# hanmekim/SceneLib2

Measured on AMD Instinct MI355X. Metric: batched MonoSLAM frames/sec (320x240, 100 feat), higher is better.
Workload: dtype f64

## Files before the change

scenelib2_amd/csrc/sl2_common.hpp:

```cpp
#pragma once
#include <hip/hip_runtime.h>

#include <cstdio>
#include <cstring>
#include <string>
#include <vector>

#include "../../include/scenelib2_amd.h"
#include "sl2_math.hpp"
#include "sl2_seq_arrays.hpp"
#include "sl2_step_plan.hpp"

namespace sl2 {

void set_error(const std::string& s);
const char* hip_err_text(hipError_t e);

#define SL2_HIP(call)                                                                          \
  do {                                                                                         \
    hipError_t _e = (call);                                                                    \
    if (_e != hipSuccess) {                                                                    \
      char _buf[512];                                                                          \
      snprintf(_buf, sizeof(_buf), "%s:%d: %s -> %s", __FILE__, __LINE__, #call, hipGetErrorString(_e)); \
      sl2::set_error(_buf);                                                                    \
      return SL2_ERR_HIP;                                                                      \
    }                                                                                          \
  } while (0)

inline int round_up(int v, int a) { return (v + a - 1) / a * a; }

enum : int {
  FF_ACTIVE = 1,
  FF_SCHEDULED = 2,
  FF_SELECTED = 4,
  FF_SUCCESS = 8,
  FF_VISIBLE = 16,
  FF_USED = 32,
  FF_PARTIAL = 64,
};

constexpr int kMaxParticles = 1024;
constexpr int kSrchSplitDefault = 8;
__host__ __device__ inline int srch_split_default(int width, int height) {
  const int frame_bands = ((width + 31) / 32) * ((height + 15) / 16);
  const int t = frame_bands * kSrchSplitDefault / 150;
  return t > kSrchSplitDefault ? t : kSrchSplitDefault;
}
constexpr int kSrchBigUnits = 16384;
constexpr int kSrchBigSlots = 64;
constexpr int kSrchBigMinBands = 4;
constexpr int kSrchSharedNu = -(1 << 30);
constexpr int kSrchBigEntries = 4;
constexpr int kSrchBigDone = kSrchBigEntries + 4 * kSrchBigUnits;
constexpr int kSrchBigParts = kSrchBigDone + kSrchBigUnits;
constexpr int kSrchBigInts = kSrchBigParts + 8 * kSrchBigUnits;
constexpr int kSeqTimeNominal = 0, kSeqTimeOwed = 1, kSeqTimeUsed = 2, kSeqTimeCatchUp = 3;
constexpr int kSeqCamFku = 0, kSeqCamFkv = 1, kSeqCamU0 = 2, kSeqCamV0 = 3, kSeqCamKd1 = 4, kSeqCamSd = 5;
static_assert(kSeqCamDoubles * sizeof(double) == 64, "one cache line per sequence");
__host__ __device__ inline int srch_unit_bands(int bands) { const int g = (bands + kSrchBigSlots - 1) / kSrchBigSlots; return g > kSrchBigMinBands ? g : kSrchBigMinBands; }
constexpr int kMaxPartial = 4;
enum : int { kPartCount = 0, kPartOrder , kPartUU = 5, kPartVV, kPartRegionValid,
             kPartRegion , kPartInitialised = 12, kPartConverted, kPartDeleted, kPartCreated };
enum : int { kPsActive = 0, kPsLabel , kPsAttempts, kPsNp, kPsMaking };
constexpr int kCholBlock = 32;
constexpr int kPatchPackedOffset = 128;

constexpr int kXcds = 8;
inline int xcd_grid(int tiles, int B) { return tiles * round_up(B, kXcds); }
#if defined(__HIPCC__)
__device__ __forceinline__ bool xcd_map(int tiles, int B, int* seq, int* tile) {
  const int L = blockIdx.x;
  const int xcd = L % kXcds, slot = L / kXcds;
  *seq = (slot / tiles) * kXcds + xcd;
  *tile = slot % tiles;
  return *seq < B;
}
#endif

#if defined(__HIPCC__)
__device__ __forceinline__ CameraParams load_cam(const double* __restrict__ seq_cam, int b, int width, int height) {
  const double* rec = seq_cam + (size_t)b * kSeqCamDoubles;
  CameraParams cam;
  cam.width = width; cam.height = height;
  cam.fku = rec[kSeqCamFku]; cam.fkv = rec[kSeqCamFkv]; cam.u0 = rec[kSeqCamU0]; cam.v0 = rec[kSeqCamV0];
  cam.kd1 = rec[kSeqCamKd1]; cam.sd = (int)rec[kSeqCamSd];
  return cam;
}
#endif

struct KernelTimer {
  std::string name;
  double total_ms = 0.0;
  int64_t launches = 0;
};
struct PendingEvent {
  int timer;
  hipEvent_t start, stop;
};

}

struct sl2_engine : sl2::SeqArrays {
  int device = 0;
  hipStream_t stream = nullptr;
  bool own_stream = false;
  sl2::CameraParams cam;
  sl2_params prm;
  int B = 0;
  int N = 0;
  int ld = 0;
  int nsel_max = 0;
  int mld = 0;
  int nblk_max = 0;
  long long steps_done = 0;
  int chol_variant = 1;
  void* chol_trace = nullptr;
  int build_variant = 1;
  int fwd_variant = 1;
  int ppos = 0;
  int kpart = 1;
  int pcap = 128;
  double* score_map = nullptr;
  int* me_big_list = nullptr;
  int* me_big_count = nullptr;
  bool mapping_used = false;
  int* init_uv = nullptr;
  struct StepGraph { const void* frames; size_t stride; sl2::StepPlan plan; hipGraphExec_t exec; };
  bool graph_mode = false;
  std::vector<StepGraph> step_graphs;
  long long graph_captures = 0;
  int build_split = 0;
  int score_threads = 0;
  int no_ksplit = 0;
  int panel_from = 16;
  int group_from = 13;
  int fwd_group = 8;
  int chol_panel = 8;
  int build_lds_min = 0;
  int search_lds_pad = 0;
  int search_chunk = 0;
  int search_variant = 1;
  int* slots_max_dev = nullptr;
  unsigned long long* slots_mail = nullptr;
  unsigned long long* slots_mail_dev = nullptr;
  unsigned long long* parts_mail = nullptr;
  unsigned long long* parts_mail_dev = nullptr;
  int place_candidates = 0;
  float place_syrk_ms[2] = {0, 0};
  float place_kept_ms[4] = {0, 0, 0, 0};
  float place_worst_ms[3] = {0, 0, 0};
  long long parts_block_step = -1;
  int slots_exact = 0;
  long long slots_exact_step = 0;
  int step_fusion = 1;
  int search_split = sl2::kSrchSplitDefault;
  int* srch_big = nullptr;
  std::vector<sl2_camera> cams_host;
  void* stats_host = nullptr;
  void* stats_host_dev = nullptr;

  void* snap_stage = nullptr;
  void* snap_host = nullptr;
  void* snap_host_dev = nullptr;
  size_t snap_cap = 0;
  unsigned long long snap_ticket = 0;
  void* snapb_stage = nullptr;
  size_t snapb_stage_bytes = 0;
  void* snapb_aux = nullptr;
  void* snapb_aux_host = nullptr;
  void* ovl_lists = nullptr;
  size_t ovl_lists_bytes = 0;
  void* ovl_images = nullptr;
  size_t ovl_images_bytes = 0;
  void* acc_dev = nullptr;
  size_t acc_dev_bytes = 0;
  void* acc_host = nullptr;
  size_t acc_host_bytes = 0;
  void* ckpt_stage = nullptr;
  size_t ckpt_stage_bytes = 0;
  hipEvent_t ckpt_event = nullptr;

  uint8_t* frames_buf = nullptr;
  const uint8_t* cur_frames = nullptr;
  size_t cur_stride = 0;

  bool profiling = false;
  int profile_level = 2;
  std::string profile_focus;
  std::vector<sl2::KernelTimer> timers;
  std::vector<sl2::PendingEvent> pending;
  std::vector<hipEvent_t> event_pool;

  sl2_engine* root = nullptr;
  std::vector<sl2_engine*> groups;
  int group_first = 0;
  hipEvent_t fork_event = nullptr;

  int timer_id(const char* name);
  void prof_begin(int id, hipStream_t st);
  void prof_end(hipStream_t st);
  int fold_events();
  int sync_all();
};

namespace sl2 {

inline const SeqArrays& seq_arrays(const sl2_engine* e) { return *e; }

struct LaunchScope {
  sl2_engine* e;
  bool on;
  size_t slot = 0;
  static bool wanted(const sl2_engine* r, const char* name, bool major) {
    if (!r->profiling) return false;
    if (r->profile_level >= 2) return true;
    if (!major) return false;
    if (r->profile_focus.empty()) return true;
    return r->profile_focus.find(std::string(",") + name + ",") != std::string::npos;
  }
  LaunchScope(sl2_engine* eng, const char* name, bool major = false) : e(eng), on(wanted(eng->root, name, major)) {
    if (on) { e->root->prof_begin(e->root->timer_id(name), e->stream); slot = e->root->pending.size() - 1; }
  }
  ~LaunchScope() {
    if (on) hipEventRecord(e->root->pending[slot].stop, e->stream);
  }
};

int launch_predict(sl2_engine* e);
int launch_feature_prediction(sl2_engine* e);
int launch_select(sl2_engine* e, int n);
int launch_search(sl2_engine* e);
int launch_search_kernel(sl2_engine* e);
int launch_search_score(sl2_engine* e);
int launch_small_front(sl2_engine* e, int n);
int launch_small_back(sl2_engine* e, int save_trajectory, int panel_w);
int launch_update(sl2_engine* e);
int launch_syrk_on(sl2_engine* e, const double* Vt, double* P);
int launch_finalize(sl2_engine* e, int save_trajectory);
int launch_mapping(sl2_engine* e, const TailPlan& tp);
int launch_manual_init(sl2_engine* e, const int* d_uv);
int launch_auto_init(sl2_engine* e);
int launch_compact_slots(sl2_engine* e, int need, bool honour_mask = false);
int checkpoint_refresh_slots(sl2_engine* e);
int checkpoint_drop_graphs(sl2_engine* e);
int checkpoint_enable_mapping(sl2_engine* e);
void release_checkpoint_staging(sl2_engine* e);
int write_grey_image(const char* path, const uint8_t* px, int w, int h);

}
```

scenelib2_amd/csrc/sl2_ekf_update.hip:

```cpp
#include "sl2_common.hpp"
#include "sl2_chol_diag.hpp"

namespace sl2 {

typedef double v4d __attribute__((ext_vector_type(4)));

__device__ __forceinline__ v4d mfma_f64(double a, double b, v4d c) {
  return __builtin_amdgcn_mfma_f64_16x16x4f64(a, b, c, 0, 0, 0);
}

#ifdef SL2_TESTING
#define SL2_EKF_TEST_SECTION 1
#include "sl2_ekf_update_testing.inc"
#undef SL2_EKF_TEST_SECTION
#endif

constexpr int kASBatch = 4;

template <int NQ, int BATCH>
__global__ void __launch_bounds__(1024) k_build_AS(const double* __restrict__ P, const double* __restrict__ f_Hx,
                                                  const double* __restrict__ f_Hy, const double* __restrict__ f_nu,
                                                  const double* __restrict__ f_R, const int* __restrict__ succ_idx,
                                                  const int* __restrict__ m_count, double* __restrict__ At,
                                                  double* __restrict__ St, const int* __restrict__ f_hcol,
                                                  const int* __restrict__ pos_err_any, int N, int ld, int mld) {
  extern __shared__ double sAt[];
  const int b = blockIdx.x;
  const int cnt = m_count[b];
  if (cnt == 0) return;
  const int m = 2 * cnt, mp = (m + 31) / 32 * 32;
  const int t = threadIdx.x;
  double* Ab = At + (size_t)b * mld * ld;
  double* Sb = St + (size_t)b * mld * mld;
  const double* Pb = P + (size_t)b * ld * ld;
  const int* sidx = succ_idx + (size_t)b * N;
  const int* hcol = (pos_err_any[b] != 0) ? f_hcol + (size_t)b * N : nullptr;
  double pc[NQ][7];
#pragma unroll
  for (int q = 0; q < NQ; ++q) {
    const int i = t + q * (int)blockDim.x;
#pragma unroll
    for (int c = 0; c < 7; ++c) pc[q][c] = (i >= ld) ? 0.0 : ((i < 13) ? Pb[(size_t)i * ld + c] : Pb[(size_t)c * ld + i]);
  }
  double hx[7], hy[3], Rn = 0.0;
  int posa = 0;
  if (t < m) {
    const int fa = sidx[t >> 1];
    const size_t fia = (size_t)b * N + fa;
    posa = hcol ? hcol[fa] : 13 + 3 * fa;
#pragma unroll
    for (int c = 0; c < 7; ++c) hx[c] = (hcol && (unsigned)(c - posa) < 3u) ? 0.0 : f_Hx[fia * 14 + (t & 1) * 7 + c];
#pragma unroll
    for (int c = 0; c < 3; ++c) hy[c] = f_Hy[fia * 6 + (t & 1) * 3 + c];
    Rn = f_R[fia];
  }
  const int nbatch = (cnt + BATCH - 1) / BATCH, per = (nbatch + (int)gridDim.y - 1) / (int)gridDim.y;
  const int jbeg = (int)blockIdx.y * per * BATCH;
  const int jend = (jbeg + per * BATCH < cnt) ? jbeg + per * BATCH : cnt;
  for (int j0 = jbeg; j0 < jend; j0 += BATCH) {
    const int nb = (jend - j0 < BATCH) ? jend - j0 : BATCH;
#pragma unroll
    for (int jj = 0; jj < BATCH; ++jj) {
      if (jj < nb) {
        const int f = sidx[j0 + jj];
        const size_t fi = (size_t)b * N + f;
        const int pos = hcol ? hcol[f] : 13 + 3 * f;
#pragma unroll
        for (int q = 0; q < NQ; ++q) {
          const int i = t + q * (int)blockDim.x;
          if (i < ld) {
            double py[3];
#pragma unroll
            for (int c = 0; c < 3; ++c)
              py[c] = Pb[(size_t)(pos + c) * ld + i];
#pragma unroll
            for (int r = 0; r < 2; ++r) {
              double acc = 0.0;
#pragma unroll
              for (int c = 0; c < 7; ++c) acc += pc[q][c] * ((hcol && (unsigned)(c - pos) < 3u) ? 0.0 : f_Hx[fi * 14 + r * 7 + c]);
#pragma unroll
              for (int c = 0; c < 3; ++c) acc += py[c] * f_Hy[fi * 6 + r * 3 + c];
              if (i == ld - 1) acc = f_nu[fi * 2 + r];
              Ab[(size_t)(2 * (j0 + jj) + r) * ld + i] = acc;
              sAt[(2 * jj + r) * ld + i] = acc;
            }
          }
        }
      }
    }
    __syncthreads();
    if (t < mp) {
#pragma unroll
      for (int kk = 0; kk < 2 * BATCH; ++kk) {
        const int k = 2 * j0 + kk;
        if (kk < 2 * nb && (t | 31) >= k) {
          double v = 0.0;
          if (t < m) {
            const double* arow = sAt + kk * ld;
            double acc = 0.0;
#pragma unroll
            for (int c = 0; c < 7; ++c) acc += hx[c] * arow[c];
#pragma unroll
            for (int c = 0; c < 3; ++c) acc += hy[c] * arow[posa + c];
            if (t == k) acc += Rn;
            v = acc;
          }
          Sb[(size_t)k * mld + t] = v;
        }
      }
    }
    __syncthreads();
  }
  if (blockIdx.y != 0) return;
  for (int k = m; k < mp; ++k) {
#pragma unroll
    for (int q = 0; q < NQ; ++q) {
      const int i = t + q * (int)blockDim.x;
      if (i < ld) Ab[(size_t)k * ld + i] = 0.0;
    }
    if (t < mp && (t | 31) >= k) Sb[(size_t)k * mld + t] = (t == k) ? 1.0 : 0.0;
  }
}


#ifdef SL2_TESTING
#define SL2_EKF_TEST_SECTION 3
#include "sl2_ekf_update_testing.inc"
#undef SL2_EKF_TEST_SECTION
#endif


__device__ __forceinline__ double fast_rcp(double p) {
  double r = __builtin_amdgcn_rcp(p);
  r = __builtin_fma(__builtin_fma(-p, r, 1.0), r, r);
  r = __builtin_fma(__builtin_fma(-p, r, 1.0), r, r);
  return r;
}
__device__ __forceinline__ double fast_rsqrt(double p) {
  double y = __builtin_amdgcn_rsq(p);
  y = y * __builtin_fma(-0.5 * p * y, y, 1.5);
  y = y * __builtin_fma(-0.5 * p * y, y, 1.5);
  return y;
}


#ifdef SL2_TESTING
#define SL2_EKF_TEST_SECTION 4
#include "sl2_ekf_update_testing.inc"
#undef SL2_EKF_TEST_SECTION
#endif

#ifdef SL2_TESTING
#define SL2_EKF_TEST_SECTION 5
#include "sl2_ekf_update_testing.inc"
#undef SL2_EKF_TEST_SECTION
#endif

#ifdef SL2_TESTING
#define SL2_EKF_TEST_SECTION 6
#include "sl2_ekf_update_testing.inc"
#undef SL2_EKF_TEST_SECTION
#endif


struct Tile32 {
  v4d f[2][2];
};

__device__ __forceinline__ Tile32 tile_load(const double* __restrict__ Sb, int mld, int k0, int i0, int lo, int hi) {
  Tile32 t;
#pragma unroll
  for (int kt = 0; kt < 2; ++kt)
#pragma unroll
    for (int it = 0; it < 2; ++it)
#pragma unroll
      for (int r = 0; r < 4; ++r) t.f[kt][it][r] = Sb[(size_t)(k0 + 16 * kt + hi + 4 * r) * mld + i0 + 16 * it + lo];
  return t;
}
__device__ __forceinline__ void tile_store(double* __restrict__ Sb, int mld, int k0, int i0, int lo, int hi, const Tile32& t) {
#pragma unroll
  for (int kt = 0; kt < 2; ++kt)
#pragma unroll
    for (int it = 0; it < 2; ++it)
#pragma unroll
      for (int r = 0; r < 4; ++r) Sb[(size_t)(k0 + 16 * kt + hi + 4 * r) * mld + i0 + 16 * it + lo] = t.f[kt][it][r];
}
constexpr int kTileAll = 15, kTileRowsLo = 5, kTileDiag = 11, kTileDiagLo = 1;
__device__ __forceinline__ Tile32 tile_panel(const double* sLinv, const double* __restrict__ Sb, int mld, int o, int i0, int lo,
                                             int hi, int need) {
  double b0[8], b1[8];
#pragma unroll
  for (int s8 = 0; s8 < 8; ++s8) {
    b0[s8] = Sb[(size_t)(o + 4 * s8 + hi) * mld + i0 + lo];
    b1[s8] = (need & 10) ? Sb[(size_t)(o + 4 * s8 + hi) * mld + i0 + 16 + lo] : 0.0;
  }
  Tile32 t;
#pragma unroll
  for (int kt = 0; kt < 2; ++kt)
#pragma unroll
    for (int it = 0; it < 2; ++it) t.f[kt][it] = (v4d){0, 0, 0, 0};
#pragma unroll
  for (int s8 = 0; s8 < 8; ++s8) {
    const int p = 4 * s8 + hi;
    const double a0 = sLinv[p * kLinvPitch + lo], a1 = sLinv[p * kLinvPitch + 16 + lo];
    t.f[0][0] = mfma_f64(a0, b0[s8], t.f[0][0]);
    if (need & 2) t.f[0][1] = mfma_f64(a0, b1[s8], t.f[0][1]);
    t.f[1][0] = mfma_f64(a1, b0[s8], t.f[1][0]);
    if (need & 8) t.f[1][1] = mfma_f64(a1, b1[s8], t.f[1][1]);
  }
  return t;
}
__device__ __forceinline__ Tile32 tile_panel_regs(const double* sLinv, const Tile32& in, int lo, int hi, int need) {
  Tile32 t;
#pragma unroll
  for (int kt = 0; kt < 2; ++kt)
#pragma unroll
    for (int it = 0; it < 2; ++it) t.f[kt][it] = (v4d){0, 0, 0, 0};
#pragma unroll
  for (int s8 = 0; s8 < 8; ++s8) {
    const int p = 4 * s8 + hi;
    const double a0 = sLinv[p * kLinvPitch + lo], a1 = sLinv[p * kLinvPitch + 16 + lo];
    const double b0 = in.f[s8 >> 2][0][s8 & 3], b1 = in.f[s8 >> 2][1][s8 & 3];
    t.f[0][0] = mfma_f64(a0, b0, t.f[0][0]);
    if (need & 2) t.f[0][1] = mfma_f64(a0, b1, t.f[0][1]);
    t.f[1][0] = mfma_f64(a1, b0, t.f[1][0]);
    if (need & 8) t.f[1][1] = mfma_f64(a1, b1, t.f[1][1]);
  }
  return t;
}
__device__ __forceinline__ void tile_trail(double* __restrict__ Sb, int mld, int o, int K, int I, int lo, int hi) {
  Tile32 acc = tile_load(Sb, mld, K * 32, I * 32, lo, hi);
#pragma unroll
  for (int h = 0; h < 2; ++h) {
    double a0[4], a1[4], b0[4], b1[4];
#pragma unroll
    for (int s4 = 0; s4 < 4; ++s4) {
      const size_t row = (size_t)(o + 16 * h + 4 * s4 + hi) * mld;
      a0[s4] = Sb[row + K * 32 + lo];
      a1[s4] = Sb[row + K * 32 + 16 + lo];
      b0[s4] = Sb[row + I * 32 + lo];
      b1[s4] = Sb[row + I * 32 + 16 + lo];
    }
#pragma unroll
    for (int s4 = 0; s4 < 4; ++s4) {
      acc.f[0][0] = mfma_f64(-a0[s4], b0[s4], acc.f[0][0]);
      acc.f[0][1] = mfma_f64(-a0[s4], b1[s4], acc.f[0][1]);
      acc.f[1][0] = mfma_f64(-a1[s4], b0[s4], acc.f[1][0]);
      acc.f[1][1] = mfma_f64(-a1[s4], b1[s4], acc.f[1][1]);
    }
  }
  tile_store(Sb, mld, K * 32, I * 32, lo, hi, acc);
}


#undef TR

__device__ __forceinline__ Tile32 tile_left_update(double* __restrict__ Sb, int mld, int J, int I, int kend, int lo, int hi, int need) {
  Tile32 acc = tile_load(Sb, mld, J * 32, I * 32, lo, hi);
  for (int K = 0; K < kend; ++K) {
#pragma unroll
    for (int h = 0; h < 2; ++h) {
      double a0[4], a1[4], b0[4], b1[4];
#pragma unroll
      for (int s4 = 0; s4 < 4; ++s4) {
        const size_t row = (size_t)(K * 32 + 16 * h + 4 * s4 + hi) * mld;
        a0[s4] = Sb[row + J * 32 + lo];
        a1[s4] = (need & 12) ? Sb[row + J * 32 + 16 + lo] : 0.0;
        b0[s4] = Sb[row + I * 32 + lo];
        b1[s4] = (need & 10) ? Sb[row + I * 32 + 16 + lo] : 0.0;
      }
#pragma unroll
      for (int s4 = 0; s4 < 4; ++s4) {
// ... 602 lines not shown
    *(double2*)&sAB[buf][0][kr * 64 + 32 + cs] = r.a1;
    *(double2*)&sAB[buf][1][kr * 64 + cs] = r.b0;
    *(double2*)&sAB[buf][1][kr * 64 + 32 + cs] = r.b1;
  };
  Stage r0 = stage_load(0);
  const int i0 = ti * 64 + wi, j0 = tj * 64 + wj;
  const int b_lo = (n_live + 31) >> 5, b_hi = ppos >> 5;
  const bool idle = ((ti == tj) && (wi > wj)) || ((i0 >> 5) >= b_lo && (i0 >> 5) < b_hi) || ((j0 >> 5) >= b_lo && (j0 >> 5) < b_hi);
  v4d acc[2][2];
  for (int it = 0; it < 2; ++it) for (int jt = 0; jt < 2; ++jt) acc[it][jt] = (v4d){0, 0, 0, 0};
  const int nchunk = mp / kSyrkKC;
  Stage r1 = r0;
  if (nchunk > 1) r1 = stage_load(1);
  const bool interior = (i0 + 32 < ld && j0 + 32 < ld);
  const bool diagw = (ti == tj) && (wi == wj) && interior;
  auto chunk_mfma = [&](int buf, int nks) {
    const int sw = (hi & 1) << 4;
    const double* pa = &sAB[buf][0][hi * 64 + wi + lo];
    const double* pb = &sAB[buf][1][hi * 64 + wj + lo];
#pragma unroll
    for (int ks = 0; ks < kSyrkKC / 4; ++ks) {
      if (ks < nks) {
        const double a0 = pa[ks * 256 + sw], a1 = pa[ks * 256 + (sw ^ 16)];
        const double b0 = pb[ks * 256 + sw], b1 = pb[ks * 256 + (sw ^ 16)];
        acc[0][0] = mfma_f64(a0, b0, acc[0][0]);
        acc[0][1] = mfma_f64(a0, b1, acc[0][1]);
        if (!diagw) acc[1][0] = mfma_f64(a1, b0, acc[1][0]);
        acc[1][1] = mfma_f64(a1, b1, acc[1][1]);
      }
    }
  };
  double pold[2][2][4];
  auto fetch_tile = [&]() {
    const double* prow = Pb + (size_t)(i0 + hi) * ld + j0 + lo;
#pragma unroll
    for (int it = 0; it < 2; ++it)
#pragma unroll
      for (int jt = 0; jt < 2; ++jt)
#pragma unroll
        for (int r = 0; r < 4; ++r) pold[it][jt][r] = prow[(size_t)(16 * it + 4 * r) * ld + 16 * jt];
  };
  const bool want_tile = !idle;
  for (int ch = 0; ch < nchunk; ch += 2) {
    stage_store(0, r0);
    __syncthreads();
    if (ch + 2 < nchunk) r0 = stage_load(ch + 2);
    if (!idle) chunk_mfma(0, (ch + 1 >= nchunk) ? nks_last : kSyrkKC / 4);
    if (ch + 1 >= nchunk) break;
    stage_store(1, r1);
    __syncthreads();
    if (ch + 3 < nchunk) r1 = stage_load(ch + 3);
    if (!idle) chunk_mfma(1, (ch + 2 >= nchunk) ? nks_last : kSyrkKC / 4);
  }
  const int lastbuf = (nchunk - 1) & 1;
  if (want_tile) fetch_tile();
  if (idle) return;
  const bool mirror = (ti != tj) || (wi != wj);
  auto plain = [&](int it, int jt) { return interior || ((i0 + 16 * it + 16 < ld) && (j0 + 16 * jt + 16 < ld)); };
  {
    double* prow = Pb + (size_t)(i0 + hi) * ld + j0 + lo;
#pragma unroll
    for (int it = 0; it < 2; ++it)
#pragma unroll
      for (int jt = 0; jt < 2; ++jt) {
        if (!plain(it, jt)) continue;
#pragma unroll
        for (int r = 0; r < 4; ++r) {
          if (diagw && it == 1 && jt == 0) continue;
          const double pn = pold[it][jt][r] - acc[it][jt][r];
          prow[(size_t)(16 * it + 4 * r) * ld + 16 * jt] = pn;
          acc[it][jt][r] = pn;
        }
      }
    if (mirror || diagw) {
      const int other = lastbuf ^ 1;
      double* sM = &sAB[other][0][0] + wave * (16 * 17);
      double* pm = Pb + (size_t)(j0 + hi) * ld + i0 + lo;
#pragma unroll
      for (int it = 0; it < 2; ++it)
#pragma unroll
        for (int jt = 0; jt < 2; ++jt) {
          if (diagw && !(it == 0 && jt == 1)) continue;
          if (!plain(it, jt)) continue;
#pragma unroll
          for (int r = 0; r < 4; ++r) sM[lo * 17 + 4 * r + hi] = acc[it][jt][r];
          asm volatile("s_waitcnt lgkmcnt(0)" ::: "memory");
#pragma unroll
          for (int k = 0; k < 4; ++k) pm[(size_t)(16 * jt + 4 * k) * ld + 16 * it] = sM[(4 * k + hi) * 17 + lo];
          asm volatile("s_waitcnt lgkmcnt(0)" ::: "memory");
        }
    }
    if (interior) return;
  }
  double* xb = x + (size_t)b * ld;
#pragma unroll
  for (int it = 0; it < 2; ++it)
#pragma unroll
    for (int jt = 0; jt < 2; ++jt) {
      if (plain(it, jt)) continue;
#pragma unroll
      for (int r = 0; r < 4; ++r) {
        const int row = i0 + 16 * it + hi + 4 * r, col = j0 + 16 * jt + lo;
        const double v = acc[it][jt][r];
        if (col == ld - 1) {
          if (row != ld - 1) xb[row] += v;
        } else if (row != ld - 1) {
          const double pn = pold[it][jt][r] - v;
          Pb[(size_t)row * ld + col] = pn;
          if (mirror) Pb[(size_t)col * ld + row] = pn;
        }
      }
    }
}

#ifdef SL2_TESTING
#define SL2_EKF_TEST_SECTION 9
#include "sl2_ekf_update_testing.inc"
#undef SL2_EKF_TEST_SECTION
#endif


static int launch_update_range(sl2_engine* e) {
  const int B = e->B;
#ifdef SL2_TESTING
  const int build_variant = e->root->build_variant, chol_variant = e->root->chol_variant, fwd_variant = e->root->fwd_variant;
#else
  const int chol_variant = 1, fwd_variant = 1;
#endif
#ifdef SL2_TESTING
  if (build_variant == 0) {
    {
      LaunchScope ls(e, "k_build_A", true);
      const int threads = e->ld <= 512 ? e->ld : 512;
      hipLaunchKernelGGL(k_build_A, dim3(B), dim3(threads), 0, e->stream, e->P, e->f_Hx, e->f_Hy, e->f_nu, e->succ_idx,
                         e->m_gate, e->At, e->N, e->ld, e->mld);
      SL2_HIP(hipGetLastError());
    }
    {
      LaunchScope ls(e, "k_build_S");
      dim3 grid(e->mld / 32, (e->mld + 255) / 256, B);
      hipLaunchKernelGGL(k_build_S, grid, dim3(256), 0, e->stream, e->At, e->f_Hx, e->f_Hy, e->f_R, e->succ_idx, e->m_gate,
                         e->St, e->N, e->ld, e->mld);
      SL2_HIP(hipGetLastError());
    }
  } else
#endif
  {
    LaunchScope ls(e, "k_build_AS", true);
    int nsplit = B >= 1024 ? 1 : (3072 + B - 1) / B;
    if (e->root->build_split > 0) nsplit = e->root->build_split;
    if (nsplit < 1) nsplit = 1;
    const int nbatch_max = (e->N + kASBatch - 1) / kASBatch;
    if (nsplit > nbatch_max) nsplit = nbatch_max;
    if (e->ld <= 1024) {
      size_t shm = sizeof(double) * 2 * kASBatch * e->ld;
      if ((size_t)e->root->build_lds_min > shm) shm = (size_t)e->root->build_lds_min;
      hipLaunchKernelGGL((k_build_AS<1, kASBatch>), dim3(B, nsplit), dim3(e->ld), shm, e->stream, e->P, e->f_Hx, e->f_Hy, e->f_nu, e->f_R,
                         e->succ_idx, e->m_gate, e->At, e->St, e->f_hcol, e->pos_err_any, e->N, e->ld, e->mld);
    } else {
      const size_t shm = sizeof(double) * 2 * 2 * e->ld;
      hipLaunchKernelGGL((k_build_AS<2, 2>), dim3(B, nsplit), dim3(1024), shm, e->stream, e->P, e->f_Hx, e->f_Hy, e->f_nu, e->f_R,
                         e->succ_idx, e->m_gate, e->At, e->St, e->f_hcol, e->pos_err_any, e->N, e->ld, e->mld);
    }
    SL2_HIP(hipGetLastError());
  }
  if (e->nblk_max > e->root->panel_from && chol_variant >= 1 && e->mld % 64 == 0 && e->nblk_max % kCholPanelBlocks == 0) {
    int rc = launch_chol_panels(e, B);
    if (rc != SL2_OK) return rc;
  } else if (e->nblk_max <= e->root->panel_from && chol_variant == 1) {
    LaunchScope ls(e, "k_chol_left", true);
    hipLaunchKernelGGL(k_chol_left, dim3(B), dim3(256), 0, e->stream, e->St, e->LinvT, e->m_gate, e->mld, e->nblk_max, 0,
                       e->nblk_max, (long long*)e->root->chol_trace);
    SL2_HIP(hipGetLastError());
  } else {
#ifdef SL2_TESTING
    {
      for (int J = 0; J < e->nblk_max; ++J) {
        {
          LaunchScope ls(e, "k_chol_diag");
          hipLaunchKernelGGL(k_chol_diag, dim3(B), dim3(64), 0, e->stream, e->St, e->LinvT, e->m_gate, e->mld, e->nblk_max, J);
          SL2_HIP(hipGetLastError());
        }
        const int rem = e->nblk_max - 1 - J;
        if (rem > 0) {
          {
            LaunchScope ls(e, "k_chol_panel");
            hipLaunchKernelGGL(k_chol_panel, dim3(rem, B), dim3(64), 0, e->stream, e->St, e->LinvT, e->m_gate, e->mld,
                               e->nblk_max, J);
            SL2_HIP(hipGetLastError());
          }
          {
            LaunchScope ls(e, "k_chol_trail");
            hipLaunchKernelGGL(k_chol_trail, dim3(rem * (rem + 1) / 2, B), dim3(64), 0, e->stream, e->St, e->m_gate, e->mld, J);
            SL2_HIP(hipGetLastError());
          }
        }
      }
    }
#else
    set_error("launch_update: no factorisation for this system size (sl2_create should have padded it)");
    return SL2_ERR_INVALID;
#endif
  }
  {
    bool done = false;
    if (fwd_variant == 1) {
      int rc = launch_fwdsub_lds(e, B, &done);
      if (rc != SL2_OK) return rc;
      if (!done && e->mld % 64 == 0) {
        rc = launch_fwdsub_grouped(e, B);
        if (rc != SL2_OK) return rc;
        done = true;
      }
    }
    if (!done) {
#ifdef SL2_TESTING
      LaunchScope ls(e, "k_fwdsub", true);
      hipLaunchKernelGGL(k_fwdsub, dim3(xcd_grid(e->ld / 64, B)), dim3(128), 0, e->stream, e->At, e->Vt, e->St, e->LinvT,
                         e->m_gate, e->ld, e->mld, e->nblk_max, B);
      SL2_HIP(hipGetLastError());
#else
      set_error("launch_update: no substitution kernel for this system size (sl2_create should have padded it)");
      return SL2_ERR_INVALID;
#endif
    }
  }
  {
    LaunchScope ls(e, "k_syrk", true);
    const int nt = e->ld / 64;
#ifdef SL2_CHOL_TRACE
    static const bool trace_syrk = getenv("SL2_TRACE_SYRK") != nullptr;
    hipLaunchKernelGGL(k_syrk, dim3(xcd_grid(nt * (nt + 1) / 2, B)), dim3(256), 0, e->stream, e->Vt, e->P, e->x, e->m_gate,
                       e->ld, e->mld, B, e->n_slots, e->ppos, trace_syrk ? (long long*)e->root->chol_trace : nullptr);
#else
    hipLaunchKernelGGL(k_syrk, dim3(xcd_grid(nt * (nt + 1) / 2, B)), dim3(256), 0, e->stream, e->Vt, e->P, e->x, e->m_gate,
                       e->ld, e->mld, B, e->n_slots, e->ppos);
#endif
    SL2_HIP(hipGetLastError());
  }
  return SL2_OK;
}

int launch_update(sl2_engine* e) { return launch_update_range(e); }

int launch_syrk_on(sl2_engine* e, const double* Vt, double* P) {
  const int nt = e->ld / 64;
#ifdef SL2_CHOL_TRACE
  hipLaunchKernelGGL(k_syrk, dim3(xcd_grid(nt * (nt + 1) / 2, e->B)), dim3(256), 0, e->stream, Vt, P, e->x, e->m_count, e->ld, e->mld, e->B,
                     e->n_slots, e->ppos, (long long*)nullptr);
#else
  hipLaunchKernelGGL(k_syrk, dim3(xcd_grid(nt * (nt + 1) / 2, e->B)), dim3(256), 0, e->stream, Vt, P, e->x, e->m_count, e->ld, e->mld, e->B,
                     e->n_slots, e->ppos);
#endif
  SL2_HIP(hipGetLastError());
  return SL2_OK;
}

}

#ifdef SL2_TESTING
#define SL2_EKF_TEST_SECTION 10
#include "sl2_ekf_update_testing.inc"
#undef SL2_EKF_TEST_SECTION
#endif
```

scenelib2_amd/csrc/sl2_engine.hip:

```cpp
#include "sl2_common.hpp"
#include "sl2_mapmath.hpp"

#include <mutex>

namespace sl2 {

static thread_local std::string g_err;
void set_error(const std::string& s) { g_err = s; }


__global__ void k_add_features(double* __restrict__ x, double* __restrict__ xp_org, uint8_t* __restrict__ patch,
                               int* __restrict__ patch_sums, int* __restrict__ f_flags, int* __restrict__ n_slots,
                               int* __restrict__ attempted, int* __restrict__ successful, int* __restrict__ f_label,
                               int* __restrict__ next_label, const double* __restrict__ y_in,
                               const double* __restrict__ xp_in, const uint8_t* __restrict__ patch_in, int seq0, int nfeat,
                               int N, int ld) {
  const int s = blockIdx.x, b = seq0 + s;
  const int base = n_slots[b];
  const int base_label = next_label[b];
  for (int f = threadIdx.x; f < nfeat; f += blockDim.x) {
    const int slot = base + f;
    const size_t fi = (size_t)b * N + slot;
    const size_t src = (size_t)s * nfeat + f;
    for (int k = 0; k < 3; ++k) x[(size_t)b * ld + 13 + 3 * slot + k] = y_in[src * 3 + k];
// ... 300 lines not shown
    for (const Cand& c : cP) { lo = c.ms < lo ? c.ms : lo; hi = c.ms > hi ? c.ms : hi; }
    return lo <= 0.93f * hi;
  };
  while ((int)cP.size() < 4 * kPlaceTries && !p_found() && rc == SL2_OK) {
    if (sizeof(double) * B * nP > budget) break;
    budget -= sizeof(double) * B * nP;
    double* p = nullptr;
    if (dmalloc(&p, B * nP) != SL2_OK) { (void)hipGetLastError(); break; }
    add(cP, p, nP);
  }
  auto by_ms = [](const Cand& x, const Cand& y) { return x.ms < y.ms; };
  std::stable_sort(cP.begin(), cP.end(), by_ms);
  std::stable_sort(cA.begin(), cA.end(), by_ms);
  std::stable_sort(cS.begin(), cS.end(), by_ms);
  size_t bp = 0, bv = 0;
  if (rc == SL2_OK && e->ld % 64 == 0) {
    std::vector<int> full_m(B, (int)(mld / 2)), full_n(B, e->N);
    hipMemcpy(e->m_count, full_m.data(), sizeof(int) * B, hipMemcpyHostToDevice);
    hipMemcpy(e->n_slots, full_n.data(), sizeof(int) * B, hipMemcpyHostToDevice);
    const size_t np4 = cP.size() < 4 ? cP.size() : 4, nv4 = cA.size() < 4 ? cA.size() : 4;
    float best = 1e30f, worst = 0.0f, best_score = 1e30f;
    hipEvent_t e0, e1;
    hipEventCreate(&e0); hipEventCreate(&e1);
    for (size_t i = 0; i < np4 && rc == SL2_OK; ++i)
      for (size_t j = 0; j < nv4 && rc == SL2_OK; ++j) {
        float t_best = 1e30f;
        for (int rep = 0; rep < 3 && rc == SL2_OK; ++rep) {
          hipEventRecord(e0, e->stream);
          rc = launch_syrk_on(e, cA[j].p, cP[i].p);
          hipEventRecord(e1, e->stream);
          if (hipEventSynchronize(e1) != hipSuccess) { set_error("placement probe failed"); rc = SL2_ERR_HIP; }
          float ms = 0.0f;
          hipEventElapsedTime(&ms, e0, e1);
          if (rep > 0 && ms < t_best) t_best = ms;
        }
        const float score = t_best + cP[i].ms;
        if (score < best_score) { best_score = score; best = t_best; bp = i; bv = j; }
        if (t_best > worst && t_best < 1e29f) worst = t_best;
      }
    hipEventDestroy(e0); hipEventDestroy(e1);
    hipMemset(e->m_count, 0, sizeof(int) * B);
    hipMemset(e->n_slots, 0, sizeof(int) * B);
    e->place_syrk_ms[0] = best; e->place_syrk_ms[1] = worst;
  }
  const size_t ba = (bv == 0) ? 1 : 0;
  e->P = cP[bp].p; e->Vt = cA[bv].p; e->At = cA[ba].p; e->St = cS[0].p;
  for (size_t i = 0; i < cP.size(); ++i) if (i != bp) hipFree(cP[i].p);
  for (size_t i = 0; i < cA.size(); ++i) if (i != bv && i != ba) hipFree(cA[i].p);
  for (size_t i = 1; i < cS.size(); ++i) hipFree(cS[i].p);
  e->place_worst_ms[0] = cP.back().ms; e->place_worst_ms[1] = cA.back().ms; e->place_worst_ms[2] = cS.back().ms;
  e->place_kept_ms[0] = cP[bp].ms; e->place_kept_ms[1] = cA[bv].ms; e->place_kept_ms[2] = cA[ba].ms; e->place_kept_ms[3] = cS[0].ms;
  e->place_candidates = (int)cP.size();
  return rc;
}

int sl2_create(const sl2_camera* cam, const sl2_params* params, int batch, int max_features, int device, void* stream,
               sl2_engine** out) {
  if (!cam || !params || !out || batch <= 0 || max_features <= 0) { set_error("sl2_create: bad argument"); return SL2_ERR_INVALID; }
  if (cam->width < 2 * SL2_PATCH_SIZE || cam->height < 2 * SL2_PATCH_SIZE) { set_error("sl2_create: image too small"); return SL2_ERR_INVALID; }
  int rc = check_device();
  if (rc != SL2_OK) return rc;
  SL2_HIP(hipSetDevice(device));
  sl2_engine* e = new sl2_engine();
  e->device = device;
  e->root = e;
  auto build = [&]() -> int {
  if (stream) { e->stream = (hipStream_t)stream; e->own_stream = false; }
  else { SL2_HIP(hipStreamCreate(&e->stream)); e->own_stream = true; }
  e->cam.width = cam->width; e->cam.height = cam->height; e->cam.fku = cam->fku; e->cam.fkv = cam->fkv;
  e->cam.u0 = cam->u0; e->cam.v0 = cam->v0; e->cam.kd1 = cam->kd1; e->cam.sd = cam->sd;
  e->prm = *params;
  if (e->prm.minimum_attempted_measurements_of_feature <= 0) e->prm.minimum_attempted_measurements_of_feature = 10;
  if (!(e->prm.successful_match_fraction > 0.0)) e->prm.successful_match_fraction = 0.5;
  e->B = batch; e->N = max_features;
  e->kpart = params->max_features_to_init_at_once < 1 ? 1 : (params->max_features_to_init_at_once > kMaxPartial ? kMaxPartial : params->max_features_to_init_at_once);
  e->search_split = srch_split_default(e->cam.width, e->cam.height);
  e->ld = round_up(13 + 3 * max_features + 6 * e->kpart + 1, 64);
  e->ppos = 13 + 3 * max_features;
  int nsel = params->number_of_features_to_select;
  if (nsel < 1) nsel = 1;
  if (nsel > max_features) nsel = max_features;
  e->nsel_max = nsel;
#ifdef SL2_TESTING
  if (const char* v = getenv("SL2_PANEL_FROM")) e->panel_from = e->group_from = atoi(v);
#endif
  e->mld = round_up(2 * nsel, 32);
  if (e->mld / 32 > e->group_from) e->mld = round_up(2 * nsel, 64);
  if (e->mld / 32 > e->panel_from) e->mld = round_up(2 * nsel, 128);
  e->nblk_max = e->mld / 32;
  {
    int np = params->number_of_particles;
    np = np < 1 ? 1 : (np > kMaxParticles ? kMaxParticles : np);
    e->pcap = round_up(np, 64);
  }
#ifndef SL2_TESTING
  if (e->ld > 2048 || e->mld > 1024) {
    set_error("sl2_create: at most 676 feature slots (2048 state columns) and 512 features measured per frame");
    return SL2_ERR_CAPACITY;
  }
#endif
  const size_t B = batch;
  {
    const size_t N = max_features, ld = e->ld, mld = e->mld, nblk_max = e->nblk_max, kpart = e->kpart, pcap = e->pcap;
#define X(type, name, elems) { const int r = dmalloc(&e->name, B * (size_t)(elems)); if (r != SL2_OK) return r; }
    SL2_SEQ_ARRAYS(X)
#undef X
  }
  SL2_HIP(hipMemset(e->active, 1, B));
  {
    std::vector<double> rec(B * kSeqTimeDoubles, 0.0);
    for (size_t b = 0; b < B; ++b) rec[b * kSeqTimeDoubles + kSeqTimeNominal] = e->prm.delta_t;
    SL2_HIP(hipMemcpy(e->seq_time, rec.data(), sizeof(double) * rec.size(), hipMemcpyHostToDevice));
  }
  {
    std::vector<double> rec(B * kSeqCamDoubles, 0.0);
    for (size_t b = 0; b < B; ++b) {
      double* c = &rec[b * kSeqCamDoubles];
      c[kSeqCamFku] = cam->fku; c[kSeqCamFkv] = cam->fkv; c[kSeqCamU0] = cam->u0; c[kSeqCamV0] = cam->v0;
      c[kSeqCamKd1] = cam->kd1; c[kSeqCamSd] = (double)cam->sd;
    }
    SL2_HIP(hipMemcpy(e->seq_cam, rec.data(), sizeof(double) * rec.size(), hipMemcpyHostToDevice));
    sl2_camera c0;
    memset(&c0, 0, sizeof(c0));
    c0.width = cam->width; c0.height = cam->height; c0.fku = cam->fku; c0.fkv = cam->fkv; c0.u0 = cam->u0; c0.v0 = cam->v0;
    c0.kd1 = cam->kd1; c0.sd = cam->sd;
    e->cams_host.assign(B, c0);
  }
  SL2_HIP(hipMalloc((void**)&e->slots_max_dev, sizeof(int) * 2));
  SL2_HIP(hipMemset(e->slots_max_dev, 0, sizeof(int) * 2));
  SL2_HIP(hipHostMalloc((void**)&e->slots_mail, 2 * sizeof(unsigned long long), hipHostMallocMapped | hipHostMallocCoherent));
  e->slots_mail[0] = 0ull; e->slots_mail[1] = 0ull;
  SL2_HIP(hipHostGetDevicePointer((void**)&e->slots_mail_dev, e->slots_mail, 0));
  e->parts_mail = e->slots_mail + 1; e->parts_mail_dev = e->slots_mail_dev + 1;
  {
    std::vector<unsigned long long> seeds(B, kRand48Seed0);
    SL2_HIP(hipMemcpy(e->rand48, seeds.data(), sizeof(unsigned long long) * B, hipMemcpyHostToDevice));
  }
  SL2_HIP(hipDeviceSynchronize());
  e->root = e;
#ifdef SL2_TESTING
  if (!getenv("SL2_NO_PLACE"))
#endif
  { int rc2 = place_large_matrices(e); if (rc2 != SL2_OK) return rc2; }
#ifdef SL2_TESTING
  if (getenv("SL2_DEBUG_PLACE")) fprintf(stderr, "PLACE %d candidates; kept P %.4f Vt %.4f At %.4f St %.4f; slowest P %.4f A %.4f St %.4f\n", e->place_candidates, e->place_kept_ms[0], e->place_kept_ms[1], e->place_kept_ms[2], e->place_kept_ms[3], e->place_worst_ms[0], e->place_worst_ms[1], e->place_worst_ms[2]);
#endif
  int G = 1;
#ifdef SL2_TESTING
  if (const char* v = getenv("SL2_FWD_VARIANT")) e->fwd_variant = atoi(v);
  if (const char* v = getenv("SL2_CHOL_VARIANT")) e->chol_variant = atoi(v);
  if (const char* v = getenv("SL2_BUILD_VARIANT")) e->build_variant = atoi(v);
  if (const char* v = getenv("SL2_SEARCH_VARIANT")) e->search_variant = atoi(v);
  if (const char* v = getenv("SL2_BUILD_SPLIT")) e->build_split = atoi(v);
  if (const char* v = getenv("SL2_SCORE_THREADS")) e->score_threads = atoi(v);
  if (getenv("SL2_NO_KSPLIT")) e->no_ksplit = 1;
  if (const char* v = getenv("SL2_SEARCH_CHUNK")) e->search_chunk = atoi(v);
  if (const char* v = getenv("SL2_SEARCH_LDS_PAD")) e->search_lds_pad = atoi(v);
  if (const char* v = getenv("SL2_BUILD_LDS_MIN")) e->build_lds_min = atoi(v);
  if (const char* v = getenv("SL2_CHOL_PANEL")) e->chol_panel = atoi(v);
  if (const char* v = getenv("SL2_FWD_GROUP")) e->fwd_group = atoi(v);
  if (const char* env = getenv("SL2_GROUPS")) if (atoi(env) > 0) G = atoi(env);
#endif
  {
    int rc2 = build_groups(e, G);
    if (rc2 != SL2_OK) return rc2;
  }
  return SL2_OK;
  };
  rc = build();
  if (rc != SL2_OK) { sl2_destroy(e); return rc; }
  *out = e;
  return SL2_OK;
}

int sl2_set_groups(sl2_engine* e, int groups) {
  if (!e || groups < 1) return SL2_ERR_INVALID;
  SL2_HIP(hipSetDevice(e->device));
  { int rc = e->sync_all(); if (rc != SL2_OK) return rc; }
  { int rc = drop_step_graphs(e); if (rc != SL2_OK) return rc; }
  return build_groups(e, groups);
}

void sl2_destroy(sl2_engine* e) {
  if (!e) return;
  hipSetDevice(e->device);
  e->sync_all();
  for (sl2_engine* g : e->groups) free_group(e, g);
  if (e->fork_event) hipEventDestroy(e->fork_event);
  for (auto& sg : e->step_graphs) hipGraphExecDestroy(sg.exec);
#define X(type, name, elems) if (e->name) hipFree(e->name);
  SL2_SEQ_ARRAYS(X)
#undef X
  void* lazy[] = {e->frames_buf, e->score_map, e->me_big_list, e->init_uv};
  for (void* p : lazy) if (p) hipFree(p);
  release_checkpoint_staging(e);
  if (e->slots_max_dev) hipFree(e->slots_max_dev);
  if (e->stats_host) hipHostFree(e->stats_host);
  if (e->slots_mail) hipHostFree(e->slots_mail);
  if (e->snap_stage) hipFree(e->snap_stage);
  if (e->snap_host) hipHostFree(e->snap_host);
  if (e->snapb_stage) hipFree(e->snapb_stage);
  if (e->snapb_aux) hipFree(e->snapb_aux);
  if (e->snapb_aux_host) hipHostFree(e->snapb_aux_host);
  if (e->ovl_lists) hipFree(e->ovl_lists);
  if (e->ovl_images) hipFree(e->ovl_images);
  if (e->acc_dev) hipFree(e->acc_dev);
  if (e->acc_host) hipHostFree(e->acc_host);
  for (auto& pe : e->pending) { hipEventDestroy(pe.start); hipEventDestroy(pe.stop); }
  for (auto ev : e->event_pool) hipEventDestroy(ev);
  if (e->own_stream) hipStreamDestroy(e->stream);
  delete e;
}

int sl2_synchronize(sl2_engine* e) {
  if (!e) return SL2_ERR_INVALID;
  { int _rc = e->sync_all(); if (_rc != SL2_OK) return _rc; }
  return SL2_OK;
}
void* sl2_get_stream(sl2_engine* e) { return e ? (void*)e->stream : nullptr; }
int sl2_batch(const sl2_engine* e) { return e ? e->B : 0; }
int sl2_max_features(const sl2_engine* e) { return e ? e->N : 0; }

static int range_ok(sl2_engine* e, int seq0, int nseq) { return e && seq0 >= 0 && nseq > 0 && seq0 + nseq <= e->B; }

static int refresh_slots_exact(sl2_engine* e) {
  std::vector<int> slots(e->B);
  SL2_HIP(hipMemcpy(slots.data(), e->n_slots, sizeof(int) * e->B, hipMemcpyDeviceToHost));
  int mx = 0;
  for (int v : slots) mx = v > mx ? v : mx;
  e->slots_exact = mx;
  e->slots_exact_step = e->steps_done;
  return SL2_OK;
}

static int slots_upper_bound(const sl2_engine* e) {
  const long long s = e->steps_done;
  const long long grow = e->mapping_used ? e->kpart : 0;
  long long best = (long long)e->slots_exact + grow * (s - e->slots_exact_step);
  const unsigned long long mail = __atomic_load_n(e->slots_mail, __ATOMIC_ACQUIRE);
  const long long t = (long long)(mail >> 32);
  if (t >= 1 && t - 1 >= e->slots_exact_step && t - 1 < s) {
    const long long viaMail = (long long)(mail & 0xffffffffull) + grow * (s - (t - 1));
    if (viaMail < best) best = viaMail;
  }
  return best > 1000000 ? 1000000 : (int)best;
}

static int parts_state_for_step(const sl2_engine* e) {
  if (e->B != 1 || !e->mapping_used || e->step_fusion == 0 || e->parts_block_step == e->steps_done || e->steps_done <= 0) return 0;
  const unsigned long long mail = __atomic_load_n(e->parts_mail, __ATOMIC_ACQUIRE);
  if ((long long)(mail >> 32) != e->steps_done) return 0;
  const long long left = (long long)(mail & 0xffffffffull);
  return left == 0 ? 1 : (left >= e->kpart ? 2 : 0);
}

int sl2_set_vehicle_state(sl2_engine* e, int seq0, int nseq, const double* xv, const double* Pxx) {
  if (!range_ok(e, seq0, nseq) || !xv || !Pxx) return SL2_ERR_INVALID;
  SL2_HIP(hipSetDevice(e->device));
  { int _rc = e->sync_all(); if (_rc != SL2_OK) return _rc; }
  const size_t nx = (size_t)13 * nseq, nP = (size_t)169 * nseq;
  { int _rc = acc_scratch(e, sizeof(double) * (nx + nP), 0); if (_rc != SL2_OK) return _rc; }
  double* dxv = (double*)e->acc_dev;
  double* dP = dxv + nx;
  SL2_HIP(hipMemcpyAsync(dxv, xv, sizeof(double) * nx, hipMemcpyHostToDevice, e->stream));
  SL2_HIP(hipMemcpyAsync(dP, Pxx, sizeof(double) * nP, hipMemcpyHostToDevice, e->stream));
  hipLaunchKernelGGL(k_set_vehicle, dim3(nseq), dim3(64), 0, e->stream, e->x, e->P, dxv, dP, seq0, e->ld);
  SL2_HIP(hipGetLastError());
  { int _rc = e->sync_all(); if (_rc != SL2_OK) return _rc; }
  return SL2_OK;
}

int sl2_get_vehicle_state(sl2_engine* e, int seq0, int nseq, double* xv, double* Pxx) {
  if (!range_ok(e, seq0, nseq) || !xv || !Pxx) return SL2_ERR_INVALID;
  SL2_HIP(hipSetDevice(e->device));
  const size_t nx = (size_t)13 * nseq, nP = (size_t)169 * nseq;
  { int _rc = acc_scratch(e, sizeof(double) * (nx + nP), sizeof(double) * (nx + nP)); if (_rc != SL2_OK) return _rc; }
  double* dxv = (double*)e->acc_dev;
  double* dP = dxv + nx;
  hipLaunchKernelGGL(k_get_vehicle, dim3(nseq), dim3(64), 0, e->stream, e->x, e->P, dxv, dP, seq0, e->ld);
  SL2_HIP(hipGetLastError());
  SL2_HIP(hipMemcpyAsync(e->acc_host, dxv, sizeof(double) * (nx + nP), hipMemcpyDeviceToHost, e->stream));
  { int _rc = e->sync_all(); if (_rc != SL2_OK) return _rc; }
  memcpy(xv, e->acc_host, sizeof(double) * nx);
  memcpy(Pxx, (const double*)e->acc_host + nx, sizeof(double) * nP);
  return SL2_OK;
}

int sl2_set_feature_covariances(sl2_engine* e, int seq0, int nseq, int nfeat, const double* Pyy) {
  if (!range_ok(e, seq0, nseq) || nfeat <= 0 || nfeat > e->N || !Pyy) return SL2_ERR_INVALID;
  SL2_HIP(hipSetDevice(e->device));
  { int _rc = e->sync_all(); if (_rc != SL2_OK) return _rc; }
  const size_t cnt = (size_t)nseq * nfeat * 9;
  { int _rc = acc_scratch(e, sizeof(double) * cnt, 0); if (_rc != SL2_OK) return _rc; }
  double* d = (double*)e->acc_dev;
  SL2_HIP(hipMemcpyAsync(d, Pyy, sizeof(double) * cnt, hipMemcpyHostToDevice, e->stream));
  hipLaunchKernelGGL(k_set_feature_cov, dim3(nseq), dim3(256), 0, e->stream, e->P, d, seq0, nfeat, e->ld);
  SL2_HIP(hipGetLastError());
  { int _rc = e->sync_all(); if (_rc != SL2_OK) return _rc; }
  return SL2_OK;
}

int sl2_add_known_features(sl2_engine* e, int seq0, int nseq, int nfeat, const double* y, const double* xp_org,
                           const uint8_t* patches) {
  if (!range_ok(e, seq0, nseq) || nfeat <= 0 || !y || !xp_org || !patches) return SL2_ERR_INVALID;
  SL2_HIP(hipSetDevice(e->device));
  { int _rc = e->sync_all(); if (_rc != SL2_OK) return _rc; }
// ... 931 lines not shown
```

Measured before the change: 1.001 million.

## Add software-pipelined A/S build kernel with prefetched P rows and LDS feature table

Adds a new k_build_AS_ahead kernel used when the build is not split and LDS fits. It stages per-feature Jacobians, innovations, noise and column positions into an LDS table once per block, then processes features in batches while prefetching the next batch's P rows into registers. This hides global load latency behind the A-row and S-column computation. In exchange it uses more registers and LDS, which may lower occupancy, and it is a new numerical code path that has to match the existing kernel exactly.

New measurement: 1.021 million, median of 6. 1.9% higher.

```diff
diff --git a/scenelib2_amd/csrc/sl2_common.hpp b/scenelib2_amd/csrc/sl2_common.hpp
--- a/scenelib2_amd/csrc/sl2_common.hpp
+++ b/scenelib2_amd/csrc/sl2_common.hpp
@@ -136,6 +136,7 @@
   int group_from = 13;
   int fwd_group = 8;
   int chol_panel = 8;
+  int build_ahead = 1;
   int build_lds_min = 0;
   int search_lds_pad = 0;
   int search_chunk = 0;
diff --git a/scenelib2_amd/csrc/sl2_ekf_update.hip b/scenelib2_amd/csrc/sl2_ekf_update.hip
--- a/scenelib2_amd/csrc/sl2_ekf_update.hip
+++ b/scenelib2_amd/csrc/sl2_ekf_update.hip
@@ -118,6 +118,174 @@
       const int i = t + q * (int)blockDim.x;
       if (i < ld) Ab[(size_t)k * ld + i] = 0.0;
     }
+    if (t < mp && (t | 31) >= k) Sb[(size_t)k * mld + t] = (t == k) ? 1.0 : 0.0;
+  }
+}
+
+constexpr int kAheadEntry = 24;
+constexpr int kAheadLdsMax = 40960;
+
+template <int BATCH>
+struct AheadRows { double v[BATCH][3]; };
+
+__device__ __forceinline__ int ahead_pos(const double* en) { return *(const int*)(en + 23); }
+
+__device__ __forceinline__ double ahead_lane(double v, int l) {
+  return __hiloint2double(__builtin_amdgcn_readlane(__double2hiint(v), l), __builtin_amdgcn_readlane(__double2loint(v), l));
+}
+
+typedef __attribute__((address_space(1))) double ahead_gdouble;
+__device__ __forceinline__ ahead_gdouble* ahead_at(const double* row, int t) {
+  unsigned long long a = (unsigned long long)row;
+  asm("" : "+s"(a));
+  return (ahead_gdouble*)(a + (unsigned)t * (unsigned)sizeof(double));
+}
+
+template <int BATCH, bool FULL>
+__device__ __forceinline__ void ahead_load(AheadRows<BATCH>& w, const double* __restrict__ Pb, const double* tab, int j0, int nb,
+                                           int ld, int t) {
+#pragma unroll
+  for (int jj = 0; jj < BATCH; ++jj) {
+    if (FULL || jj < nb) {
+      const int pos = __builtin_amdgcn_readfirstlane(ahead_pos(tab + (j0 + jj) * kAheadEntry));
+#pragma unroll
+      for (int c = 0; c < 3; ++c) w.v[jj][c] = *ahead_at(Pb + (size_t)(pos + c) * ld, t);
+    }
+  }
+}
+
+template <int BATCH, bool FULL, bool REFILL>
+__device__ __forceinline__ void ahead_rows(AheadRows<BATCH>& w, const double (&pc)[7], const double* tab, const double* __restrict__ Pb,
+                                           double* __restrict__ Ab, double* sAt, int j0, int nb, int ld, int t) {
+#pragma unroll
+  for (int jj = 0; jj < BATCH; ++jj) {
+    if (FULL || jj < nb) {
+      double en = 0.0;
+      if ((t & 63) < kAheadEntry) en = tab[(j0 + jj) * kAheadEntry + (t & 63)];
+#pragma unroll
+      for (int r = 0; r < 2; ++r) {
+        double acc = 0.0;
+#pragma unroll
+        for (int c = 0; c < 7; ++c) acc += pc[c] * ahead_lane(en, r * 7 + c);
+#pragma unroll
+        for (int c = 0; c < 3; ++c) acc += w.v[jj][c] * ahead_lane(en, 14 + r * 3 + c);
+        if (t == ld - 1) acc = ahead_lane(en, 20 + r);
+        *ahead_at(Ab + (size_t)(2 * (j0 + jj) + r) * ld, t) = acc;
+        sAt[(2 * jj + r) * ld + t] = acc;
+      }
+      if (REFILL && jj < BATCH - 1) {
+        const int pos = __builtin_amdgcn_readfirstlane(ahead_pos(tab + (j0 + BATCH + jj) * kAheadEntry));
+#pragma unroll
+        for (int c = 0; c < 3; ++c) w.v[jj][c] = *ahead_at(Pb + (size_t)(pos + c) * ld, t);
+      }
+    }
+  }
+}
+
+template <int BATCH>
+__device__ __forceinline__ void ahead_refill_last(AheadRows<BATCH>& w, const double* tab, const double* __restrict__ Pb, int j0, int ld, int t) {
+  const int pos = __builtin_amdgcn_readfirstlane(ahead_pos(tab + (j0 + 2 * BATCH - 1) * kAheadEntry));
+#pragma unroll
+  for (int c = 0; c < 3; ++c) w.v[BATCH - 1][c] = *ahead_at(Pb + (size_t)(pos + c) * ld, t);
+}
+
+template <int BATCH>
+__device__ __forceinline__ void ahead_S(const double* sAt, const double* tab, double* __restrict__ Sb, int j0, int nb, int m, int mp,
+                                        int ld, int mld, int t) {
+  __syncthreads();
+  double hx[7], hy[3], Rn = 0.0;
+  int posa = 0;
+  if (t < m) {
+    const double* en = tab + (t >> 1) * kAheadEntry;
+#pragma unroll
+    for (int c = 0; c < 7; ++c) hx[c] = en[(t & 1) * 7 + c];
+#pragma unroll
+    for (int c = 0; c < 3; ++c) hy[c] = en[14 + (t & 1) * 3 + c];
+    Rn = en[22];
+    posa = ahead_pos(en);
+  }
+#pragma unroll
+  for (int kk = 0; kk < 2 * BATCH; ++kk) {
+    const int k = 2 * j0 + kk;
+    if (kk < 2 * nb) {
+      const double* arow = sAt + kk * ld;
+      if (t < mp && (t | 31) >= k) {
+        double v = 0.0;
+        if (t < m) {
+          double acc = 0.0;
+#pragma unroll
+          for (int c = 0; c < 7; ++c) acc += hx[c] * arow[c];
+#pragma unroll
+          for (int c = 0; c < 3; ++c) acc += hy[c] * arow[posa + c];
+          if (t == k) acc += Rn;
+          v = acc;
+        }
+        Sb[(size_t)k * mld + t] = v;
+      }
+    }
+  }
+  __syncthreads();
+}
+
+template <int BATCH>
+__global__ void __launch_bounds__(1024) __attribute__((amdgpu_waves_per_eu(6, 8))) k_build_AS_ahead(const double* __restrict__ P, const double* __restrict__ f_Hx,
+                                                        const double* __restrict__ f_Hy, const double* __restrict__ f_nu,
+                                                        const double* __restrict__ f_R, const int* __restrict__ succ_idx,
+                                                        const int* __restrict__ m_count, double* __restrict__ At,
+                                                        double* __restrict__ St, const int* __restrict__ f_hcol,
+                                                        const int* __restrict__ pos_err_any, int N, int ld, int mld, int tab_cap) {
+  extern __shared__ double sAt[];
+  const int b = blockIdx.x;
+  int cnt = m_count[b];
+  if (cnt == 0) return;
+  cnt = cnt > tab_cap ? tab_cap : cnt;
+  const int m = 2 * cnt, mp = (m + 31) / 32 * 32;
+  const int t = threadIdx.x;
+  double* Ab = At + (size_t)b * mld * ld;
+  double* Sb = St + (size_t)b * mld * mld;
+  const double* Pb = P + (size_t)b * ld * ld;
+  double* tab = sAt + 2 * BATCH * ld;
+  {
+    const int* sidx = succ_idx + (size_t)b * N;
+    const int* hcol = (pos_err_any[b] != 0) ? f_hcol + (size_t)b * N : nullptr;
+    for (int idx = t; idx < cnt * kAheadEntry; idx += (int)blockDim.x) {
+      const int j = idx / kAheadEntry, el = idx - j * kAheadEntry;
+      const int f = sidx[j];
+      const size_t fi = (size_t)b * N + f;
+      const int pos = hcol ? hcol[f] : 13 + 3 * f;
+      double v;
+      if (el < 14) v = (hcol && (unsigned)(el % 7 - pos) < 3u) ? 0.0 : f_Hx[fi * 14 + el];
+      else if (el < 20) v = f_Hy[fi * 6 + (el - 14)];
+      else if (el < 22) v = f_nu[fi * 2 + (el - 20)];
+      else if (el == 22) v = f_R[fi];
+      else v = __longlong_as_double((long long)pos);
+      tab[idx] = v;
+    }
+  }
+  double pc[7];
+#pragma unroll
+  for (int c = 0; c < 7; ++c) pc[c] = (t < 13) ? Pb[(size_t)t * ld + c] : Pb[(size_t)c * ld + t];
+  __syncthreads();
+  const int nfull = cnt / BATCH, rem = cnt - nfull * BATCH;
+  AheadRows<BATCH> w;
+  if (nfull > 0) {
+    ahead_load<BATCH, true>(w, Pb, tab, 0, BATCH, ld, t);
+    int k = 0;
+    for (; k + 1 < nfull; ++k) {
+      ahead_rows<BATCH, true, true>(w, pc, tab, Pb, Ab, sAt, k * BATCH, BATCH, ld, t);
+      ahead_S<BATCH>(sAt, tab, Sb, k * BATCH, BATCH, m, mp, ld, mld, t);
+      ahead_refill_last<BATCH>(w, tab, Pb, k * BATCH, ld, t);
+    }
+    ahead_rows<BATCH, true, false>(w, pc, tab, Pb, Ab, sAt, k * BATCH, BATCH, ld, t);
+    ahead_S<BATCH>(sAt, tab, Sb, k * BATCH, BATCH, m, mp, ld, mld, t);
+  }
+  if (rem > 0) {
+    ahead_load<BATCH, false>(w, Pb, tab, nfull * BATCH, rem, ld, t);
+    ahead_rows<BATCH, false, false>(w, pc, tab, Pb, Ab, sAt, nfull * BATCH, rem, ld, t);
+    ahead_S<BATCH>(sAt, tab, Sb, nfull * BATCH, rem, m, mp, ld, mld, t);
+  }
+  for (int k = m; k < mp; ++k) {
+    Ab[(size_t)k * ld + t] = 0.0;
     if (t < mp && (t | 31) >= k) Sb[(size_t)k * mld + t] = (t == k) ? 1.0 : 0.0;
   }
 }
@@ -1026,7 +1194,22 @@
     if (nsplit < 1) nsplit = 1;
     const int nbatch_max = (e->N + kASBatch - 1) / kASBatch;
     if (nsplit > nbatch_max) nsplit = nbatch_max;
-    if (e->ld <= 1024) {
+    int ahead = 0;
+    if (nsplit == 1 && e->ld <= 1024 && e->root->build_ahead != 0) {
+      const size_t tab = sizeof(double) * kAheadEntry * e->nsel_max;
+      if (sizeof(double) * 2 * 4 * e->ld + tab <= (size_t)kAheadLdsMax) ahead = 4;
+      else if (sizeof(double) * 2 * 2 * e->ld + tab <= (size_t)kAheadLdsMax) ahead = 2;
+    }
+    if (ahead) {
+      size_t shm = sizeof(double) * (2 * ahead * e->ld + kAheadEntry * e->nsel_max);
+      if ((size_t)e->root->build_lds_min > shm) shm = (size_t)e->root->build_lds_min;
+      if (ahead == 4)
+        hipLaunchKernelGGL((k_build_AS_ahead<4>), dim3(B), dim3(e->ld), shm, e->stream, e->P, e->f_Hx, e->f_Hy, e->f_nu, e->f_R,
+                           e->succ_idx, e->m_gate, e->At, e->St, e->f_hcol, e->pos_err_any, e->N, e->ld, e->mld, e->nsel_max);
+      else
+        hipLaunchKernelGGL((k_build_AS_ahead<2>), dim3(B), dim3(e->ld), shm, e->stream, e->P, e->f_Hx, e->f_Hy, e->f_nu, e->f_R,
+                           e->succ_idx, e->m_gate, e->At, e->St, e->f_hcol, e->pos_err_any, e->N, e->ld, e->mld, e->nsel_max);
+    } else if (e->ld <= 1024) {
       size_t shm = sizeof(double) * 2 * kASBatch * e->ld;
       if ((size_t)e->root->build_lds_min > shm) shm = (size_t)e->root->build_lds_min;
       hipLaunchKernelGGL((k_build_AS<1, kASBatch>), dim3(B, nsplit), dim3(e->ld), shm, e->stream, e->P, e->f_Hx, e->f_Hy, e->f_nu, e->f_R,
diff --git a/scenelib2_amd/csrc/sl2_engine.hip b/scenelib2_amd/csrc/sl2_engine.hip
--- a/scenelib2_amd/csrc/sl2_engine.hip
+++ b/scenelib2_amd/csrc/sl2_engine.hip
@@ -476,6 +476,7 @@
   if (const char* v = getenv("SL2_BUILD_VARIANT")) e->build_variant = atoi(v);
   if (const char* v = getenv("SL2_SEARCH_VARIANT")) e->search_variant = atoi(v);
   if (const char* v = getenv("SL2_BUILD_SPLIT")) e->build_split = atoi(v);
+  if (const char* v = getenv("SL2_BUILD_AHEAD")) e->build_ahead = atoi(v);
   if (const char* v = getenv("SL2_SCORE_THREADS")) e->score_threads = atoi(v);
   if (getenv("SL2_NO_KSPLIT")) e->no_ksplit = 1;
   if (const char* v = getenv("SL2_SEARCH_CHUNK")) e->search_chunk = atoi(v);
```
